# ChicyChen/LOCO-Edit

Hardware: AMD Instinct MI355X
Metric: edit-directions/sec (top-5 PMP-Jacobian SVD @256^2) + vT cos-sim vs ref (higher is better)
Workload: dtype bf16x3 (split-bf16 MFMA operands, fp32 accumulate + fp32 storage); 1 GPU; CelebA-HQ DDPM 256x256 top-5 local basis (l_eye-sized mask, L=2400), t=0.6T, 12 power iterations, one GPU; multi_gpu_form=single, probes_total=5, probes_per_gpu=5, kept=5, n_iter=12, mask_L=2400, weights=synthetic seed 0, streams=2

## Files before the change

### include/loco_hip.h

```cpp
#ifndef LOCO_HIP_H
#define LOCO_HIP_H

#include <stdint.h>

#ifdef __cplusplus
extern "C" {
#endif

typedef struct loco_ctx loco_ctx;

typedef struct loco_unet_cfg {
    int32_t struct_size;
    int32_t resolution;
    int32_t in_channels;
    int32_t out_ch;
    int32_t ch;
    int32_t num_levels;
    int32_t ch_mult[8];
    int32_t num_res_blocks;
    int32_t num_attn_res;
    int32_t attn_resolutions[8];
    int32_t gn_groups;
    float   gn_eps;
    int32_t max_batch;
// ... 33 lines not shown
int  loco_sched_step(loco_ctx* ctx, const float* x, const float* et, float at, float at_next,
                     float eta, const float* noise, int64_t count, float* x_next, float* x0_out,
                     void* stream);

int  loco_pmp_primal(loco_ctx* ctx, const float* x, float t, float at,
                     const uint8_t* mask, int32_t use_et, void* stream);
int  loco_pmp_set_second_mask(loco_ctx* ctx, const uint8_t* mask2, int32_t from_row, void* stream);
int  loco_pmp_jvp(loco_ctx* ctx, const float* V, int32_t k, float* U, void* stream);
int  loco_pmp_vjp(loco_ctx* ctx, const float* U, int32_t k, float* A, void* stream);

int  loco_orthonormalize(loco_ctx* ctx, float* A, int32_t k, int64_t n, float* s, void* stream);
int  loco_qr_rows(loco_ctx* ctx, float* A, int32_t k, int64_t n, void* stream);
int  loco_convergence(loco_ctx* ctx, const float* Vprev, const float* V, int64_t count,
                      float atol, float* out2, void* stream);
int  loco_convergence_rows(loco_ctx* ctx, const float* Vprev, const float* V, int32_t k, int64_t n,
                           float atol, float* out2, void* stream);

int  loco_null_project(loco_ctx* ctx, const float* Vm, int32_t k, const float* Vn, int32_t k0,
                       int64_t n, float* out, void* stream);
int  loco_edit_axpy(loco_ctx* ctx, const float* x, const float* v, const float* alphas,
                    int32_t B, int64_t n, float* out, void* stream);
int  loco_mask_gather(loco_ctx* ctx, const float* U, int32_t k, float* out, void* stream);
int64_t loco_mask_count(loco_ctx* ctx);

int  loco_clock_stamp(loco_ctx* ctx, uint64_t* out2, void* stream);

double loco_unet_flops(loco_ctx* ctx);
int64_t loco_workspace_bytes(loco_ctx* ctx);

int  loco_timer_start(loco_ctx* ctx, void* stream);
int  loco_timer_stop(loco_ctx* ctx, void* stream, float* ms);

int  loco_set_precision(loco_ctx* ctx, int32_t mode);
int  loco_set_streams(loco_ctx* ctx, int32_t n);
int  loco_set_side_stream(loco_ctx* ctx, void* stream);
int  loco_set_chip_share(loco_ctx* ctx, int32_t n);
int  loco_get_precision(loco_ctx* ctx);

int  loco_set_cond(loco_ctx* ctx, const float* emb_add, void* stream);
int  loco_set_time_cond(loco_ctx* ctx, const float* w_emb, void* stream);
int  loco_masked_axpby(loco_ctx* ctx, const float* V, const float* E, float cv, float ce, int32_t k, float* out,
                       void* stream);
int  loco_latent_sample(loco_ctx* ctx, const float* moments, const float* noise, float scale, int32_t B, float* z, void* stream);
int  loco_set_context(loco_ctx* ctx, const float* tokens, void* stream);

int  loco_lincomb(loco_ctx* ctx, const float* const* src, const float* coef, int32_t n, float* out, int64_t count,
// ... 147 lines not shown
```

### loco-edit_amd/csrc/engine.hip

```cpp
#include <hip/hip_runtime.h>

#include <algorithm>
#include <array>
#include <cmath>
#include <cstdio>
#include <cstdlib>
#include <cstring>
#include <map>
#include <memory>
#include <thread>
#include <atomic>
#include <string>
#include <vector>

#include "../../include/loco_hip.h"
#ifdef LOCO_DIAG
#include "../../include/loco_hip_diag.h"
#endif
#include "kernels.h"
#include "program.h"
#ifdef LOCO_DIAG
#include "conv_plan_text.h"
#endif

using namespace loco;


#define HIPCHK(ctx, call)                                                                    \
    do {                                                                                     \
        hipError_t e_ = (call);                                                              \
        if (e_ != hipSuccess) {                                                              \
            (ctx)->err = std::string(#call) + ": " + hipGetErrorString(e_);                  \
            return -1;                                                                       \
        }                                                                                    \
    } while (0)

namespace {

struct ConvP {
    float* wf = nullptr;
    float* wd = nullptr;
    float* wbf = nullptr;
// ... 77 lines not shown
    double *G = nullptr, *Q = nullptr, *W = nullptr, *gscratch = nullptr;
    float* alphas = nullptr;
    float* ctx_colbias = nullptr;
    bool has_ctx = false;
    float* cond_add = nullptr;
    float* ctx_norm = nullptr;
    bool has_cond = false;
    float* cond_in = nullptr;
    bool has_tcond = false;
    float2* sxcache = nullptr;
    int prec = 0;
    std::vector<float*> owned;
    size_t bytes = 0;

    bool primal_ok = false;
    float p_cv = 0.f, p_ce = 0.f;
    uint8_t* mask = nullptr;
    bool has_mask = false;
    uint8_t* mask2 = nullptr;
    bool has_mask2 = false;
    int mask2_from = 0;
    int* mask_idx = nullptr;
    int* mask_L_dev = nullptr;
    long mask_L = 0;
    hipStream_t mask_stream = nullptr;
    int primal_B = 0;
    hipEvent_t ev0 = nullptr, ev1 = nullptr;
    int n_streams = 1;
    hipStream_t st2 = nullptr;
    hipStream_t st2_user = nullptr;
    hipEvent_t ev_fork = nullptr, ev_join = nullptr;
    double* red2 = nullptr;
    struct FwdGraph { hipGraph_t graph = nullptr; hipGraphExec_t exec = nullptr; int calls = 0; };
    std::map<int, FwdGraph> fwd_graphs;
    bool graph_on = false;
    bool gemm_lowp = true;
    unsigned char* gemm_ws[2] = {nullptr, nullptr}; size_t gemm_ws_bytes[2] = {0, 0}; int lane = 0;
    loco_ctx* weights_of = nullptr;
    int forks = 0;
    bool zombie = false;
    bool fuse_lin = true;
    int lanes_active = 1;
    int lane_s0 = 0;
    int chip_share = 1;
    hipStream_t cap_st = nullptr;
    float* xin_buf = nullptr;
// ... 362 lines not shown
    if (c->prec >= 1 && c->gemm_lowp && gemm_prefers_bf16x3(g)) launch_gemm_bf16x3(g, st); else launch_gemm(g, st);
}

void conv_defaults(ConvArgs& a) {
    std::memset(&a, 0, sizeof(a));
    a.stride = 1; a.pad = 1; a.nsplit = 1; a.mode = CM_NONE; a.res_scale = 1.f;
}

struct NS { float *sc, *sh, *mr, *tst, *tc; };
NS nstats(const loco_ctx* c, float* base, const NormP& n) {
    NS s;
    s.sc = base + n.soff; s.sh = s.sc + n.C; s.mr = s.sh + n.C; s.tst = s.mr + 2 * c->cfg.gn_groups;
    s.tc = s.tst + 2 * c->cfg.gn_groups;
    return s;
}

struct StatReq {
    int kind = ST_NONE;
    NormP* n = nullptr;
    float* stats = nullptr;
    const float* prim = nullptr;
    const float* ss_scale = nullptr; const float* ss_shift = nullptr;
    float* keep = nullptr; size_t keep_floats = 0; int* keep_ntile = nullptr;
};

void stats_standalone(loco_ctx* c, const StatReq& rq, const float* x, long xbs, int B, int HW, int s0, hipStream_t st) {
    const NormP& n = *rq.n;
    const long SB = c->prog->stats_per_sample;
    const int G = c->cfg.gn_groups;
    if (rq.kind == ST_FWD) {
        NS s = nstats(c, rq.stats + (long)s0 * SB, n);
        launch_gn_stats(x, xbs, B, n.C, HW, G, eps_of(c, n), n.gamma, n.beta, s.mr, s.sc, s.sh, SB, c->red, st, rq.ss_scale,
                        rq.ss_shift);
    } else {
        NS sp = nstats(c, c->statsP, n);
        NS stt = nstats(c, rq.stats + (long)s0 * SB, n);
        launch_gn_tstats(x, xbs, rq.prim, 0, B, n.C, HW, G, sp.sc, sp.sh, sp.mr, 0, 0, rq.kind == ST_TAN ? 0 : 1, stt.tst,
                         stt.tc, SB, c->red, st, c->cfg.act);
    }
}

bool run_conv(loco_ctx* c, const ConvArgs& a0, int taps, hipStream_t st, const StatReq* rq = nullptr,
              const ConvArgs* second = nullptr) {
    const size_t span = (size_t)c->cfg.max_batch * c->prog->per_sample;
    auto padded = [&](const float* p) { return (p >= c->arenaP && p < c->arenaP + span) || (p >= c->arenaT && p < c->arenaT + span); };
    ConvArgs a = a0, sc;
    a.act = c->cfg.act;
    if (a.mode == CM_GN_SILU && c->cfg.act == ACT_GELU) a.mode = CM_GN_GELU;
    a.in_padded = padded(a.in);
    if (second) { sc = *second; sc.in_padded = padded(sc.in); }
    ConvEnv e;
    e.prec = c->prec; e.chip_share = c->chip_share; e.lanes = c->lanes_active; e.lane_s0 = c->lane_s0;
    e.partial = c->partial; e.partial_floats = c->partial_floats; e.stpart = c->stpart; e.stpart_floats = c->stpart_floats;
    e.fuse_stats = c->fuse_stats; e.fuse_lin = c->fuse_lin; e.deep1 = c->deep1; e.max_batch = c->cfg.max_batch;
    StatAsk q;
    if (rq) {
        q.kind = rq->kind; q.norm = rq->n != nullptr; q.prim = rq->prim; q.keep = rq->keep; q.keep_floats = rq->keep_floats;
        if (rq->n && rq->n->sx_off >= 0 && c->sxcache) q.sx = c->sxcache + rq->n->sx_off;
    }
    const ConvPlan p = plan_conv(e, a, taps, rq ? &q : nullptr, second ? &sc : nullptr);
    if (p.sc_first) run_conv(c, *second, 1, st);
#ifdef LOCO_DIAG
    if (c->plan_log) conv_plan_text(p, taps, c->prec, *c->plan_log);
#endif
    if (rq && rq->kind != ST_NONE && rq->n) rq->n->ready = true;
    if (rq && rq->keep_ntile) *rq->keep_ntile = p.keep_ntile;
    const int HWo = a.Hout * a.Wout, Gn = c->cfg.gn_groups;
    const long SBs = c->prog->stats_per_sample;
    auto timed = [&](const char* name, double flops, const ConvArgs& y, auto&& launch) {
        loco_ctx::ProfRec r;
        if (c->prof_on) {
            r.name = name; r.flops = flops;
            r.cin = y.Cin; r.cout = y.Cout; r.h = y.Hout; r.b = y.B; r.ns = y.nsplit; r.mode = y.mode; r.taps = taps;
            r.e0 = c->next_event(); r.e1 = c->next_event();
            (void)hipEventRecord(r.e0, st);
        }
        launch();
        if (c->prof_on) { (void)hipEventRecord(r.e1, st); c->prof.push_back(r); }
    };
    for (int li = 0; li < p.nl; ++li) {
        const ConvLaunch& l = p.l[li];
// ... 459 lines not shown
                a.out = p.T(op.out); a.out_bs = p.bs(); a.Cout = to.C; a.Hout = to.H; a.Wout = to.W; a.B = B;
                const StatReq rq = next_fwd(op.out);
                run_conv(c, a, 9, st, &rq);
                break;
            }
            case OP_OUT: {
                const Tens& ti = c->tens[op.in];
                if (!op.n1.ready) gn_forward_stats(p, op.n1, p.T(op.in), p.bs(), ti.H * ti.W);
                op.n1.ready = false;
                NS s = nstats(c, stats, op.n1);
                ConvArgs a; conv_defaults(a);
                a.in = p.T(op.in); a.in_bs = p.bs(); a.Cin = ti.C; a.Hin = ti.H; a.Win = ti.W;
                setw(a, op.conv, false); a.bias = op.conv.bias;
                a.mode = CM_GN_SILU; a.sc = s.sc; a.sh = s.sh; a.scsh_bs = SB;
                a.out = p.T(op.out); a.out_bs = p.bs(); a.Cout = to.C; a.Hout = to.H; a.Wout = to.W; a.B = B;
                run_conv(c, a, 9, st);
                break;
            }
        }
    }
    return 0;
}

void tangent_stats(loco_ctx* c, const NormP& n, const float* d, long dbs, const float* x, int HW, int B,
                   hipStream_t st) {
    NS sp = nstats(c, c->statsP, n);
    NS stt = nstats(c, c->statsT, n);
    launch_gn_tstats(d, dbs, x, 0, B, n.C, HW, c->cfg.gn_groups, sp.sc, sp.sh, sp.mr, 0, 0, 0, stt.tst,
                     stt.tc, c->prog->stats_per_sample, c->red, st);
}
void set_tan(loco_ctx* c, ConvArgs& a, const NormP& n, const float* prim) {
    NS sp = nstats(c, c->statsP, n);
    NS stt = nstats(c, c->statsT, n);
    a.mode = CM_TAN_SILU; a.prim = prim; a.prim_bs = 0;
    a.sc = sp.sc; a.sh = sp.sh; a.scsh_bs = 0; a.mr = sp.mr; a.mr_bs = 0; a.gamma_ = n.gamma;
    a.tst = stt.tst; a.tst_bs = c->prog->stats_per_sample; a.cpg = n.C / c->cfg.gn_groups;
    a.tc = stt.tc; a.tc_bs = c->prog->stats_per_sample;
    a.sx = (n.sx_off >= 0 && c->sxcache) ? c->sxcache + n.sx_off : nullptr;
}

constexpr size_t RED_BYTES = (size_t)4 << 20;

int tangent_pass(loco_ctx* c, const float* V, int B, hipStream_t st) {
    const loco_unet_cfg& cfg = c->cfg;
    const long PS = c->prog->per_sample;
    auto TP = [&](int id) { return c->arenaP + c->tens[id].off; };
// ... 145 lines not shown
                lin1x1(c, op.pj_out, false, XT_(X_H3), PS, C, TT(op.out), PS, C, H, W, B, TT(op.in), PS, false, st, &rq);
                break;
            }
            case OP_DOWN: case OP_UP: {
                const Tens& ti = c->tens[op.in];
                ConvArgs a; conv_defaults(a);
                a.in = TT(op.in); a.in_bs = PS; a.Cin = ti.C; a.Hin = ti.H; a.Win = ti.W;
                setw(a, op.conv, false);
                if (op.kind == OP_DOWN) { a.stride = 2; a.pad = op.sym_down ? 1 : 0; } else { a.upsample = 1; }
                a.out = TT(op.out); a.out_bs = PS; a.Cout = to.C; a.Hout = to.H; a.Wout = to.W; a.B = B;
                const StatReq rq = next_tan(op.out);
                run_conv(c, a, 9, st, &rq);
                break;
            }
            case OP_OUT: {
                const Tens& ti = c->tens[op.in];
                if (!op.n1.ready) tangent_stats(c, op.n1, TT(op.in), PS, TP(op.in), ti.H * ti.W, B, st);
                op.n1.ready = false;
                ConvArgs a; conv_defaults(a);
                a.in = TT(op.in); a.in_bs = PS; a.Cin = ti.C; a.Hin = ti.H; a.Win = ti.W;
                setw(a, op.conv, false);
                set_tan(c, a, op.n1, TP(op.in));
                a.out = TT(op.out); a.out_bs = PS; a.Cout = to.C; a.Hout = to.H; a.Wout = to.W; a.B = B;
                run_conv(c, a, 9, st);
                break;
            }
        }
    }
    return 0;
}

void cot_stats(loco_ctx* c, const NormP& n, const float* d, long dbs, const float* x, int HW, int B, int kind,
               hipStream_t st) {
    NS sp = nstats(c, c->statsP, n);
    NS stt = nstats(c, c->statsT, n);
    launch_gn_tstats(d, dbs, x, 0, B, n.C, HW, c->cfg.gn_groups, sp.sc, sp.sh, sp.mr, 0, 0, kind, stt.tst,
                     stt.tc, c->prog->stats_per_sample, c->red, st, c->cfg.act);
}

int cotangent_pass(loco_ctx* c, const float* ge, const float* gx0, float* Aout, int B, hipStream_t st) {
    const loco_unet_cfg& cfg = c->cfg;
    const long PS = c->prog->per_sample;
    const int G = cfg.gn_groups;
    auto TP = [&](int id) { return c->arenaP + c->tens[id].off; };
    auto TG = [&](int id) { return c->arenaT + c->tens[id].off; };
    auto GO = [&](const Op& o) -> const float* { return o.out == c->prog->eps_t ? ge : TG(o.out); };
    auto GOS = [&](const Op& o) -> long { return o.out == c->prog->eps_t ? (long)c->prog->n_out : PS; };
    clear_ready(c);
    for (int oi = (int)c->ops.size() - 1; oi >= 0; --oi) {
        Op& op = c->ops[oi];
        const Tens& to = c->tens[op.out];
        const int HW = to.H * to.W;
        switch (op.kind) {
            case OP_OUT: {
                const Tens& ti = c->tens[op.in];
                ConvArgs a; conv_defaults(a);
                a.in = GO(op); a.in_bs = GOS(op); a.Cin = to.C; a.Hin = to.H; a.Win = to.W;
                setw(a, op.conv, true);
                a.out = TG(op.a1); a.out_bs = PS; a.Cout = ti.C; a.Hout = ti.H; a.Wout = ti.W; a.B = B;
                {
                    const StatReq rq = req_lin(c, ST_COT, &op.n1, TP(op.in));
                    run_conv(c, a, 9, st, &rq);
                    op.n1.ready = false;
                }
                NS sp = nstats(c, c->statsP, op.n1);
                NS stt = nstats(c, c->statsT, op.n1);
                launch_gn_apply(2, TG(op.a1), PS, TP(op.in), 0, nullptr, 0, TG(op.in), PS, 0, B, ti.C, ti.H * ti.W, G,
                                sp.sc, sp.sh, sp.mr, 0, 0, stt.tst, c->prog->stats_per_sample, st, cfg.act);
                break;
            }
            case OP_UP: {
                const Tens& ti = c->tens[op.in];
                ConvArgs a; conv_defaults(a);
                a.in = TG(op.out); a.in_bs = PS; a.Cin = to.C; a.Hin = to.H; a.Win = to.W;
                setw(a, op.conv, true);
                a.out = TG(op.up); a.out_bs = PS; a.Cout = ti.C; a.Hout = to.H; a.Wout = to.W; a.B = B;
                run_conv(c, a, 9, st);
                launch_pool2x2_sum(TG(op.up), PS, TG(op.in), PS, 0, B, ti.C, ti.H, ti.W, st);
                break;
            }
            case OP_DOWN: {
                const Tens& ti = c->tens[op.in];
// ... 253 lines not shown
    }
    c->partial_floats = (size_t)64 << 20;
    if (dalloc(c, &c->partial, c->partial_floats)) return -1;
    if (dalloc(c, &c->xin_buf, MB * c->prog->n_in) || dalloc(c, &c->t_dev, 4)) return -1;
    if (dalloc(c, &c->eps_buf, MB * c->prog->n_out) || dalloc(c, &c->gx0, MB * c->prog->n_in) || dalloc(c, &c->ge, MB * c->prog->n_out))
        return -1;
    if (dalloc(c, &c->tmpA, (size_t)64 * c->prog->n_in)) return -1;
    if (dalloc(c, &c->G, 64 * 64) || dalloc(c, &c->Q, 64 * 64) || dalloc(c, &c->W, SOLVER_W_GATE + 1)) return -1;
    {
        size_t nblk = ((size_t)c->prog->n_in + 255) / 256;
        if (dalloc(c, &c->gscratch, nblk * 64 * 64 + 4096)) return -1;
    }
    if (dalloc(c, &c->alphas, 256) || dalloc(c, &c->cond_add, (size_t)cfg->ch * 4)) return -1;
    if (dalloc(c, &c->cond_in, (size_t)cfg->ch)) return -1;
    {
        float2* sx0 = nullptr;
        if (dalloc(c, &sx0, (size_t)c->prog->sx_total + 64)) return -1;
        c->sxcache = sx0 + 32;
    }
    {
        const char* e = getenv("LOCO_PRECISION");
        c->prec = (e && std::string(e) == "f32") ? 0 : (e && std::string(e) == "f16") ? 2 : 1;
    }
    if (dalloc(c, &c->mask2, (size_t)c->prog->n_out)) return -1;
    if (dalloc(c, &c->mask, (size_t)c->prog->n_out) || dalloc(c, &c->mask_idx, (size_t)c->prog->n_out) ||
        dalloc(c, &c->mask_L_dev, 4)) return -1;
    HIPCHK(c, hipEventCreate(&c->ev0));
    HIPCHK(c, hipEventCreate(&c->ev1));
    {
        const char* e = getenv("LOCO_STREAMS");
        c->n_streams = (e && atoi(e) == 2) ? 2 : 1;
        HIPCHK(c, hipStreamCreateWithFlags(&c->st2, hipStreamNonBlocking));
        HIPCHK(c, hipStreamCreateWithFlags(&c->cap_st, hipStreamNonBlocking));
        const char* gl = getenv("LOCO_GEMM_LOWP");
        if (gl) c->gemm_lowp = atoi(gl) != 0;
        const char* gr = getenv("LOCO_GRAPH");
        c->graph_on = gr && atoi(gr) == 1;
        HIPCHK(c, hipEventCreateWithFlags(&c->ev_fork, hipEventDisableTiming));
        HIPCHK(c, hipEventCreateWithFlags(&c->ev_join, hipEventDisableTiming));
    }
    return 0;
}

}

extern "C" {

const char* loco_version(void) { return "loco_hip 0.2 (gfx950; conv arithmetic: f32 MFMA | bf16x3 split-bf16 MFMA | f16 MFMA)"; }

// ... 141 lines not shown

int loco_sched_step(loco_ctx* c, const float* x, const float* et, float at, float at_next, float eta,
                    const float* noise, int64_t count, float* x_next, float* x0_out, void* stream) {
    if (!c) return -2;
    if (eta != 0.f && !noise) { c->err = "eta != 0 needs a noise tensor"; return -2; }
    float s1, s2, s3, ce, cn;
    sched_coeffs(at, at_next, eta, &s1, &s2, &s3, &ce, &cn);
    launch_ddim_step(x, et, eta == 0.f ? nullptr : noise, x_next, x0_out, (long)count, s2, s1, s3, ce, cn,
                     (hipStream_t)stream);
    HIPCHK(c, hipGetLastError());
    return 0;
}

int loco_ddim_step(loco_ctx* c, const float* x, float t, float at, float at_next, float eta, const float* noise,
                   int32_t B, float* x_next, void* stream) {
    if (!c) return -2;
    if (eta != 0.f && !noise) { c->err = "eta != 0 needs a noise tensor"; return -2; }
    if (c->prog->n_out != c->prog->n_in) { c->err = "loco_ddim_step: this network is not a denoiser (output and input sizes differ)"; return -2; }
    int rc = loco_unet_forward(c, x, t, B, c->eps_buf, stream);
    if (rc) return rc;
    return loco_sched_step(c, x, c->eps_buf, at, at_next, eta, noise, (int64_t)B * c->prog->n_in, x_next, nullptr, stream);
}

int loco_pmp_primal(loco_ctx* c, const float* x, float t, float at, const uint8_t* mask, int32_t use_et,
                    void* stream) {
    if (!c) return -2;
    if (finalize_params(c)) return -3;
    if (c->prog->n_out != c->prog->n_in && !use_et) {
        c->err = "loco_pmp_primal: a network whose output size differs from its input has no x0 combination; use_et = 1 "
                 "(raw network Jacobian)";
        return -2;
    }
    hipStream_t st = (hipStream_t)stream;
    if (forward_pass(c, x, t, 1, c->arenaP, c->statsP, st)) return -1;
    c->primal_B = 1;
    if (c->prec >= 1) {
        for (auto& op : c->ops) {
            if (op.kind != OP_RES && op.kind != OP_OUT) continue;
            const Tens& ti = c->tens[op.in];
            const int HW = ti.H * ti.W, G = c->cfg.gn_groups;
            NS s1 = nstats(c, c->statsP, op.n1);
            launch_gn_cache(c->arenaP + ti.off, op.n1.C, HW, op.n1.C / G, s1.sc, s1.sh, s1.mr,
                            c->sxcache + op.n1.sx_off, st, c->cfg.act);
            if (op.kind == OP_RES) {
                const Tens& th = c->tens[op.h1];
                NS s2 = nstats(c, c->statsP, op.n2);
                launch_gn_cache(c->arenaP + th.off, op.n2.C, th.H * th.W, op.n2.C / G, s2.sc, s2.sh, s2.mr,
                                c->sxcache + op.n2.sx_off, st, c->cfg.act);
            }
        }
    }
    if (use_et) { c->p_cv = 0.f; c->p_ce = 1.f; }
    else { c->p_cv = 1.0f / std::sqrt(at); c->p_ce = -std::sqrt(1.0f - at) / std::sqrt(at); }
    c->has_mask = (mask != nullptr);
    c->has_mask2 = false;
    c->mask_L = c->prog->n_out;
    if (mask) {
        HIPCHK(c, hipMemcpyAsync(c->mask, mask, (size_t)c->prog->n_out, hipMemcpyDeviceToDevice, st));
        launch_mask_compact(c->mask, c->prog->n_out, c->mask_idx, c->mask_L_dev, st);
        c->mask_L = -1;
        c->mask_stream = st;
    }
    HIPCHK(c, hipGetLastError());
    c->primal_ok = true;
    return 0;
}

int loco_pmp_set_second_mask(loco_ctx* c, const uint8_t* mask2, int32_t from_row, void* stream) {
    if (!c) return -2;
    if (!c->primal_ok) { c->err = "loco_pmp_primal has not been called"; return -2; }
    if (!mask2) { c->has_mask2 = false; return 0; }
    if (!c->has_mask) { c->err = "a second mask needs a first one (loco_pmp_primal with mask)"; return -2; }
    if (from_row < 0) { c->err = "from_row must be >= 0"; return -2; }
    HIPCHK(c, hipMemcpyAsync(c->mask2, mask2, (size_t)c->prog->n_out, hipMemcpyDeviceToDevice, (hipStream_t)stream));
    c->has_mask2 = true;
    c->mask2_from = from_row;
    return 0;
}

int loco_pmp_jvp(loco_ctx* c, const float* V, int32_t k, float* U, void* stream) {
    if (!c) return -2;
    if (!c->primal_ok) { c->err = "loco_pmp_primal has not been called"; return -2; }
    hipStream_t st = (hipStream_t)stream;
    const int MB = c->cfg.max_batch;
    for (int b0 = 0; b0 < k; b0 += MB) {
        int B = (k - b0 < MB) ? k - b0 : MB;
        int rc = run_lanes(c, B, st, [&](int s0, int nb, hipStream_t ls) -> int {
            const float* Vc = V + (long)(b0 + s0) * c->prog->n_in;
            if (tangent_pass(c, Vc, nb, ls)) return -1;
            launch_copy(c->arenaT + c->tens[c->prog->eps_t].off, c->prog->per_sample, c->eps_buf, c->prog->n_out, 0, nb, c->prog->n_out, ls);
            launch_masked_axpby(c->prog->n_out == c->prog->n_in ? Vc : nullptr, c->eps_buf, c->has_mask ? c->mask : nullptr, c->p_cv,
                                c->p_ce, U + (long)(b0 + s0) * c->prog->n_out, nb, c->prog->n_out, ls,
                                c->has_mask2 ? c->mask2 : nullptr, (long)c->mask2_from - (b0 + s0));
            return 0;
        });
        if (rc) return rc;
    }
    HIPCHK(c, hipGetLastError());
    return 0;
// ... 636 lines not shown
```

### loco-edit_amd/csrc/kernels.h

```cpp
#pragma once
#include <hip/hip_runtime.h>
#include <stdint.h>

namespace loco {

struct DeviceOnce { bool seen[64] = {}; };
inline bool first_on_device(DeviceOnce& f) {
    int d = 0;
    (void)hipGetDevice(&d);
    d &= 63;
    if (f.seen[d]) return false;
    f.seen[d] = true;
    return true;
}


enum ConvMode : int {
    CM_NONE = 0,
    CM_GN_SILU = 1,
    CM_GN = 2,
    CM_TAN_SILU = 3,
    CM_COT_SILU = 4,
    CM_GN_GELU = 5,
};
// ... 241 lines not shown
                       hipStream_t st, const double* gate = nullptr);
constexpr int SOLVER_W_GATE = 64;
constexpr double SOLVER_W_FLOOR = 0x1p-47;
constexpr double SOLVER_REORTHO_RATIO = 1e-7;
void launch_jacobi_eig(double* G, int k, double* w, double* Q, hipStream_t st);
void launch_rotate_rows(const float* Ain, float* Aout, int k, long n, const double* Q, const double* w,
                        int mode, hipStream_t st);
void launch_sign_fix(float* A, int k, long n, float* s_out, const double* w, float* scratch, hipStream_t st);
void launch_cholesky(double* G, int k, hipStream_t st, double drop_below = 0.0, double* w = nullptr,
                     const double* gate = nullptr);
void launch_trsm_rows(const float* Ain, float* Aout, int k, long n, const double* L, hipStream_t st,
                      const double* gate = nullptr);
void launch_convergence(const float* a, const float* b, long count, float atol, float rtol, float* out2,
                        double* scratch, hipStream_t st);
void launch_convergence_rows(const float* a, const float* b, int k, long n, float atol, float rtol, float* out2,
                             double* scratch, hipStream_t st);
void launch_project_rows(const float* Vm, int k, const float* Vn, int k0, long n, const double* C,
                         float* out, hipStream_t st);
void launch_normalize_rows(float* A, int k, long n, double* scratch, hipStream_t st);
void launch_edit_axpy(const float* x, const float* v, const float* alphas_dev, int B, long n, float* out,
                      hipStream_t st);
void launch_mask_gather(const float* U, const int* idx, long L, long n, int k, float* out, hipStream_t st);
void launch_mask_compact(const uint8_t* mask, long n, int* idx, int* count, hipStream_t st);

}
```

### loco-edit_amd/csrc/misc.hip

```cpp
#include "kernels.h"

namespace loco {

typedef float f32x4_t __attribute__((ext_vector_type(4)));

__device__ __forceinline__ double wave_sum(double v) {
#pragma unroll
    for (int o = 32; o > 0; o >>= 1) v += __shfl_down(v, o, 64);
    return v;
}
__device__ __forceinline__ float wave_sumf(float v) {
#pragma unroll
    for (int o = 32; o > 0; o >>= 1) v += __shfl_down(v, o, 64);
    return v;
}
__device__ __forceinline__ float wave_maxf(float v) {
#pragma unroll
    for (int o = 32; o > 0; o >>= 1) v = fmaxf(v, __shfl_down(v, o, 64));
    return v;
}
__device__ __forceinline__ double block_sum(double v, double* sm) {
    v = wave_sum(v);
    __syncthreads();
    if ((threadIdx.x & 63) == 0) sm[threadIdx.x >> 6] = v;
// ... 826 lines not shown
}

__global__ void copy_kernel(const float* in, long in_bs, float* out, long out_bs, int accumulate, long per) {
    const int b = blockIdx.y;
    for (long i = ((long)blockIdx.x * blockDim.x + threadIdx.x) * 4; i < per; i += (long)gridDim.x * blockDim.x * 4) {
        float4 v = *reinterpret_cast<const float4*>(in + (long)b * in_bs + i);
        float4* o = reinterpret_cast<float4*>(out + (long)b * out_bs + i);
        if (accumulate) {
            float4 w = *o;
            v.x += w.x; v.y += w.y; v.z += w.z; v.w += w.w;
        }
        *o = v;
    }
}
void launch_copy(const float* in, long in_bs, float* out, long out_bs, int accumulate, int B, long per_sample,
                 hipStream_t st) {
    int blocks = (int)((per_sample / 4 + 255) / 256);
    if (blocks > 2048) blocks = 2048;
    if (blocks < 1) blocks = 1;
    hipLaunchKernelGGL(copy_kernel, dim3(blocks, B), dim3(256), 0, st, in, in_bs, out, out_bs, accumulate,
                       per_sample);
}

__global__ void ddim_step_kernel(const float* x, const float* eps, const float* noise, float* out, float* x0_out,
                                 long count, float sq1mat, float sqat, float sqatn, float ce, float cn) {
    for (long i = (long)blockIdx.x * blockDim.x + threadIdx.x; i < count; i += (long)gridDim.x * blockDim.x) {
        float e = eps[i];
        float p = (x[i] - e * sq1mat) / sqat;
        float v = sqatn * p + ce * e;
        if (noise) v += cn * noise[i];
        if (x0_out) x0_out[i] = p;
        out[i] = v;
    }
}
void launch_ddim_step(const float* x, const float* eps, const float* noise, float* out, float* x0_out, long count,
                      float c_x0_x, float c_x0_e, float c_next_x0, float c_next_e, float c_noise, hipStream_t st) {
    int blocks = (int)((count + 255) / 256);
    if (blocks > 2048) blocks = 2048;
    hipLaunchKernelGGL(ddim_step_kernel, dim3(blocks), dim3(256), 0, st, x, eps, noise, out, x0_out, count, c_x0_e, c_x0_x,
                       c_next_x0, c_next_e, c_noise);
}

__global__ void masked_axpby_kernel(const float* V, const float* dE, const uint8_t* mask, float cv, float ce,
                                    float* U, long n, long total, const uint8_t* mask2, long split) {
    for (long i = (long)blockIdx.x * blockDim.x + threadIdx.x; i < total; i += (long)gridDim.x * blockDim.x) {
        long row = i / n, j = i - row * n;
// ... 99 lines not shown
```

### loco-edit_amd/csrc/solver.hip

```cpp
#include "kernels.h"

namespace loco {

constexpr int GCH = 256;

__device__ __forceinline__ double wsum(double v) {
#pragma unroll
    for (int o = 32; o > 0; o >>= 1) v += __shfl_down(v, o, 64);
    return v;
}

__global__ __launch_bounds__(256) void cross_gram_partial(const float* A, int k1, const float* B, int k2, long n,
                                                          double* part, const double* gate) {
    extern __shared__ float sm[];
    if (gate && *gate == 0.0) return;
    float* As = sm;
    float* Bs = sm + (long)k1 * (GCH + 1);
    const long c0 = (long)blockIdx.x * GCH;
    for (int e = threadIdx.x; e < k1 * GCH; e += 256) {
        int i = e / GCH, c = e % GCH;
        As[i * (GCH + 1) + c] = (c0 + c < n) ? A[(long)i * n + c0 + c] : 0.f;
    }
    if (B != A) {
        for (int e = threadIdx.x; e < k2 * GCH; e += 256) {
// ... 463 lines not shown
    const long per = (n + 1023) / 1024;
    const long lo = (long)t * per, hi = lo + per < n ? lo + per : n;
    int cnt = 0;
    for (long i = lo; i < hi; ++i) cnt += mask[i] != 0;
    int inc = cnt;
#pragma unroll
    for (int o = 1; o < 64; o <<= 1) {
        int v = __shfl_up(inc, o, 64);
        if (lane >= o) inc += v;
    }
    if (lane == 63) wtot[wv] = inc;
    __syncthreads();
    int base = 0;
    for (int w = 0; w < wv; ++w) base += wtot[w];
    int pos = base + inc - cnt;
    for (long i = lo; i < hi; ++i)
        if (mask[i]) idx[pos++] = (int)i;
    if (t == 1023) *count = base + inc;
}
void launch_mask_compact(const uint8_t* mask, long n, int* idx, int* count, hipStream_t st) {
    hipLaunchKernelGGL(mask_compact_kernel, dim3(1), dim3(1024), 0, st, mask, n, idx, count);
}

}
```

### loco-edit_amd/hip.py

```python
from __future__ import annotations

import ctypes as C
import os
from typing import Dict, Optional

import numpy as np
import torch

from .config import UNetConfig

_LIB_PATH = os.environ.get("LOCO_HIP_LIB") or os.path.join(os.path.dirname(os.path.abspath(__file__)), "libloco_hip.so")
_lib = None

DIAG_SYMBOLS = ["loco_bench_conv", "loco_debug_conv", "loco_debug_tensor"]

SYMBOLS = [
    "loco_version", "loco_device_count", "loco_create", "loco_fork", "loco_destroy", "loco_last_error",
    "loco_load_param", "loco_params_missing", "loco_unet_forward", "loco_ddim_step", "loco_sched_step",
    "loco_pmp_primal", "loco_pmp_set_second_mask", "loco_pmp_jvp", "loco_pmp_vjp", "loco_orthonormalize", "loco_qr_rows",
    "loco_convergence", "loco_convergence_rows", "loco_null_project", "loco_edit_axpy", "loco_mask_gather", "loco_mask_count",
    "loco_unet_flops", "loco_workspace_bytes", "loco_clock_stamp", "loco_set_side_stream", "loco_timer_start", "loco_timer_stop",
    "loco_profile_enable", "loco_profile_report", "loco_set_precision", "loco_get_precision", "loco_set_streams", "loco_set_chip_share",
    "loco_set_cond", "loco_set_context", "loco_lincomb", "loco_masked_axpby", "loco_latent_sample",
    "loco_text_create", "loco_text_load_param", "loco_text_params_missing", "loco_text_encode", "loco_text_last_error",
    "loco_text_destroy", "loco_t5_create", "loco_text_encode_masked",
    "loco_diffedit_mask", "loco_cfg_masked_step", "loco_set_time_cond", "loco_lcm_step",
    "loco_sam_create", "loco_sam_load_param", "loco_sam_params_missing", "loco_sam_encode", "loco_sam_profile",
    "loco_sam_profile_read", "loco_sam_last_error", "loco_sam_destroy",
    "loco_samdec_create", "loco_samdec_load_param", "loco_samdec_params_missing", "loco_samdec_set_image", "loco_samdec_predict",
    "loco_samdec_score", "loco_samdec_binarize", "loco_samdec_last_error", "loco_samdec_destroy",
    "loco_clipvis_create", "loco_clipvis_load_param", "loco_clipvis_params_missing", "loco_clipvis_preprocess",
    "loco_clipvis_encode", "loco_clipvis_last_error", "loco_clipvis_destroy",
    "loco_quality_create", "loco_quality_load_param", "loco_quality_params_missing", "loco_quality_lpips", "loco_quality_ssim",
    "loco_quality_masked_mse", "loco_quality_last_error", "loco_quality_destroy",
]

DIFFEDIT_RULES = {"reference": 0, "intended": 1}


class LocoCfg(C.Structure):
    _fields_ = [
        ("struct_size", C.c_int32), ("resolution", C.c_int32), ("in_channels", C.c_int32), ("out_ch", C.c_int32), ("ch", C.c_int32),
        ("num_levels", C.c_int32), ("ch_mult", C.c_int32 * 8), ("num_res_blocks", C.c_int32),
# ... 76 lines not shown
        lib.loco_fork.argtypes = [vp, C.c_int32, C.POINTER(vp)]
    lib.loco_destroy.argtypes = [vp]
    lib.loco_destroy.restype = None
    lib.loco_last_error.argtypes = [vp]
    lib.loco_last_error.restype = C.c_char_p
    lib.loco_load_param.argtypes = [vp, C.c_char_p, vp, C.POINTER(i64), i32, i32]
    lib.loco_params_missing.argtypes = [vp]
    lib.loco_unet_forward.argtypes = [vp, vp, f32, i32, vp, vp]
    lib.loco_ddim_step.argtypes = [vp, vp, f32, f32, f32, f32, vp, i32, vp, vp]
    lib.loco_sched_step.argtypes = [vp, vp, vp, f32, f32, f32, vp, i64, vp, vp, vp]
    lib.loco_pmp_primal.argtypes = [vp, vp, f32, f32, vp, i32, vp]
    lib.loco_pmp_set_second_mask.argtypes = [vp, vp, i32, vp]
    lib.loco_pmp_jvp.argtypes = [vp, vp, i32, vp, vp]
    lib.loco_pmp_vjp.argtypes = [vp, vp, i32, vp, vp]
    lib.loco_orthonormalize.argtypes = [vp, vp, i32, i64, vp, vp]
    lib.loco_qr_rows.argtypes = [vp, vp, i32, i64, vp]
    lib.loco_convergence.argtypes = [vp, vp, vp, i64, f32, vp, vp]
    lib.loco_convergence_rows.argtypes = [vp, vp, vp, i32, i64, f32, vp, vp]
    lib.loco_null_project.argtypes = [vp, vp, i32, vp, i32, i64, vp, vp]
    lib.loco_edit_axpy.argtypes = [vp, vp, vp, C.POINTER(f32), i32, i64, vp, vp]
    lib.loco_mask_gather.argtypes = [vp, vp, i32, vp, vp]
    lib.loco_mask_count.argtypes = [vp]
    lib.loco_mask_count.restype = i64
    lib.loco_clock_stamp.argtypes = [vp, vp, vp]
    lib.loco_set_side_stream.argtypes = [vp, vp]
    lib.loco_unet_flops.argtypes = [vp]
    lib.loco_unet_flops.restype = C.c_double
    lib.loco_workspace_bytes.argtypes = [vp]
    lib.loco_workspace_bytes.restype = i64
    lib.loco_timer_start.argtypes = [vp, vp]
    lib.loco_timer_stop.argtypes = [vp, vp, C.POINTER(f32)]
    lib.loco_set_precision.argtypes = [vp, i32]
    lib.loco_get_precision.argtypes = [vp]
    lib.loco_set_streams.argtypes = [vp, i32]
    lib.loco_set_chip_share.argtypes = [vp, i32]
    lib.loco_set_cond.argtypes = [vp, vp, vp]
    lib.loco_set_context.argtypes = [vp, vp, vp]
    lib.loco_masked_axpby.argtypes = [vp, vp, vp, f32, f32, i32, vp, vp]
    lib.loco_latent_sample.argtypes = [vp, vp, vp, f32, i32, vp, vp]
    lib.loco_lincomb.argtypes = [vp, C.POINTER(vp), C.POINTER(f32), i32, vp, i64, vp]
    lib.loco_diffedit_mask.argtypes = [vp, vp, vp, f32, i32, i32, i64, i32, vp, vp, vp]
    lib.loco_cfg_masked_step.argtypes = [vp, vp, vp, vp, vp, f32, f32, f32, vp, i32, i64, vp, vp]
    lib.loco_set_time_cond.argtypes = [vp, vp, vp]
    lib.loco_lcm_step.argtypes = [vp, vp, vp, f32, f32, f32, f32, vp, i64, vp, vp, vp]
    lib.loco_profile_enable.argtypes = [vp, i32]
    lib.loco_profile_report.argtypes = [vp, C.c_char_p, i64]
# ... 293 lines not shown
    def edit_axpy(self, x, v, alphas) -> torch.Tensor:
        _chk_dev(x)
        _chk_dev(v)
        B = len(alphas)
        n = x.numel()
        out = torch.empty((B,) + tuple(x.shape[1:]), device=x.device, dtype=torch.float32)
        arr = (C.c_float * B)(*[float(a) for a in alphas])
        self._check(self.lib.loco_edit_axpy(self._ctx, _ptr(x), _ptr(v), arr, B, n, _ptr(out), _stream()),
                    "loco_edit_axpy")
        torch.cuda.current_stream().synchronize()
        return out

    def mask_gather(self, U) -> torch.Tensor:
        _chk_dev(U)
        k = U.shape[0]
        L = int(self.lib.loco_mask_count(self._ctx))
        out = torch.empty(k, L, device=U.device, dtype=torch.float32)
        self._check(self.lib.loco_mask_gather(self._ctx, _ptr(U), k, _ptr(out), _stream()), "loco_mask_gather")
        return out

    def mask_count(self) -> int:
        return int(self.lib.loco_mask_count(self._ctx))

    def set_cond(self, emb_add: Optional[torch.Tensor]):
        if emb_add is not None:
            _chk_dev(emb_add)
            if emb_add.numel() != 4 * self.cfg.ch:
                raise ValueError("conditioning embedding must have 4*ch elements")
        self._check(self.lib.loco_set_cond(self._ctx, _ptr(emb_add), _stream()), "loco_set_cond")

    def set_time_cond(self, w_emb: Optional[torch.Tensor]):
        if w_emb is not None:
            _chk_dev(w_emb)
            if self.cfg.time_cond_proj_dim > 0 and w_emb.numel() != self.cfg.time_cond_proj_dim:
                raise ValueError(f"guidance-scale embedding must have time_cond_proj_dim = {self.cfg.time_cond_proj_dim} "
                                 f"elements, got {tuple(w_emb.shape)}")
        self._check(self.lib.loco_set_time_cond(self._ctx, _ptr(w_emb), _stream()), "loco_set_time_cond")
        if w_emb is not None:
            torch.cuda.current_stream().synchronize()

    def set_context(self, tokens: torch.Tensor):
        _chk_dev(tokens)
        if tuple(tokens.shape) != (self.cfg.context_len, self.cfg.context_dim):
            raise ValueError(f"context must be [{self.cfg.context_len}, {self.cfg.context_dim}], got {tuple(tokens.shape)}")
        self._check(self.lib.loco_set_context(self._ctx, _ptr(tokens), _stream()), "loco_set_context")
        torch.cuda.current_stream().synchronize()
# ... 544 lines not shown
```

Before: 19.79 edit-directions/s.

## Restrict final output conv JVP/VJP to a window around the mask bounding box

Computes the mask's bounding box once after the primal pass and picks an aligned square window (H/4 or H/2) covering it plus a one-pixel halo. The last output conv in the tangent (JVP) and cotangent (VJP) passes then runs only on that window: inputs, primal activations and split-precision caches are copied into it, and the results are scattered back. For the VJP, GroupNorm tangent stats are rescaled by the window-to-full-area ratio and a windowed GN-backward apply kernel fills the full tensor. This removes full-resolution work on the costly final conv at the price of extra copies, a host sync during primal setup, and some numerical risk in the stats rescaling.

```diff
diff --git a/include/loco_hip.h b/include/loco_hip.h
--- a/include/loco_hip.h
+++ b/include/loco_hip.h
@@ -79,6 +79,7 @@
                     int32_t B, int64_t n, float* out, void* stream);
 int  loco_mask_gather(loco_ctx* ctx, const float* U, int32_t k, float* out, void* stream);
 int64_t loco_mask_count(loco_ctx* ctx);
+int  loco_mask_window(loco_ctx* ctx, int32_t out[3]);
 
 int  loco_clock_stamp(loco_ctx* ctx, uint64_t* out2, void* stream);
 
diff --git a/loco-edit_amd/csrc/engine.hip b/loco-edit_amd/csrc/engine.hip
--- a/loco-edit_amd/csrc/engine.hip
+++ b/loco-edit_amd/csrc/engine.hip
@@ -18,6 +18,7 @@
 #include "../../include/loco_hip_diag.h"
 #endif
 #include "kernels.h"
+#include "mask_window.h"
 #include "program.h"
 #ifdef LOCO_DIAG
 #include "conv_plan_text.h"
@@ -141,6 +142,10 @@
     int mask2_from = 0;
     int* mask_idx = nullptr;
     int* mask_L_dev = nullptr;
+    MaskWindow win;
+    float* win_buf = nullptr; size_t win_floats = 0;
+    float *win_prim = nullptr, *win_big = nullptr, *win_small = nullptr;
+    float2* win_sx = nullptr;
     long mask_L = 0;
     hipStream_t mask_stream = nullptr;
     int primal_B = 0;
@@ -549,6 +554,7 @@
     const float* prim = nullptr;
     const float* ss_scale = nullptr; const float* ss_shift = nullptr;
     float* keep = nullptr; size_t keep_floats = 0; int* keep_ntile = nullptr;
+    const float2* sx = nullptr;
 };
 
 void stats_standalone(loco_ctx* c, const StatReq& rq, const float* x, long xbs, int B, int HW, int s0, hipStream_t st) {
@@ -570,7 +576,10 @@
 bool run_conv(loco_ctx* c, const ConvArgs& a0, int taps, hipStream_t st, const StatReq* rq = nullptr,
               const ConvArgs* second = nullptr) {
     const size_t span = (size_t)c->cfg.max_batch * c->prog->per_sample;
-    auto padded = [&](const float* p) { return (p >= c->arenaP && p < c->arenaP + span) || (p >= c->arenaT && p < c->arenaT + span); };
+    auto padded = [&](const float* p) {
+        return (p >= c->arenaP && p < c->arenaP + span) || (p >= c->arenaT && p < c->arenaT + span) ||
+               (c->win_buf && p >= c->win_buf && p < c->win_buf + c->win_floats);
+    };
     ConvArgs a = a0, sc;
     a.act = c->cfg.act;
     if (a.mode == CM_GN_SILU && c->cfg.act == ACT_GELU) a.mode = CM_GN_GELU;
@@ -583,7 +592,8 @@
     StatAsk q;
     if (rq) {
         q.kind = rq->kind; q.norm = rq->n != nullptr; q.prim = rq->prim; q.keep = rq->keep; q.keep_floats = rq->keep_floats;
-        if (rq->n && rq->n->sx_off >= 0 && c->sxcache) q.sx = c->sxcache + rq->n->sx_off;
+        if (rq->sx) q.sx = rq->sx;
+        else if (rq->n && rq->n->sx_off >= 0 && c->sxcache) q.sx = c->sxcache + rq->n->sx_off;
     }
     const ConvPlan p = plan_conv(e, a, taps, rq ? &q : nullptr, second ? &sc : nullptr);
     if (p.sc_first) run_conv(c, *second, 1, st);
@@ -1089,6 +1099,10 @@
     return 0;
 }
 
+inline bool window_on(const loco_ctx* c, const Op& op) {
+    return c->win.S > 0 && !c->has_mask2 && op.kind == OP_OUT && op.out == c->prog->eps_t && &op == &c->ops.back();
+}
+
 void tangent_stats(loco_ctx* c, const NormP& n, const float* d, long dbs, const float* x, int HW, int B,
                    hipStream_t st) {
     NS sp = nstats(c, c->statsP, n);
@@ -1280,6 +1294,19 @@
                 setw(a, op.conv, false);
                 set_tan(c, a, op.n1, TP(op.in));
                 a.out = TT(op.out); a.out_bs = PS; a.Cout = to.C; a.Hout = to.H; a.Wout = to.W; a.B = B;
+                if (window_on(c, op)) {
+                    const MaskWindow& w = c->win;
+                    const long in_ws = (long)ti.C * w.S * w.S, out_ws = (long)to.C * w.S * w.S;
+                    float* tin = c->win_big + c->lane_s0 * in_ws;
+                    float* tout = c->win_small + c->lane_s0 * out_ws;
+                    launch_window_copy(1, TT(op.in), PS, tin, in_ws, B, ti.C, ti.H, ti.W, w.y0, w.x0, w.S, w.S, st);
+                    a.in = tin; a.in_bs = in_ws; a.Hin = a.Win = w.S;
+                    a.prim = c->win_prim; if (a.sx) a.sx = c->win_sx;
+                    a.out = tout; a.out_bs = out_ws; a.Hout = a.Wout = w.S;
+                    run_conv(c, a, 9, st);
+                    launch_window_copy(0, tout, out_ws, TT(op.out), PS, B, to.C, to.H, to.W, w.y0, w.x0, w.S, w.S, st);
+                    break;
+                }
                 run_conv(c, a, 9, st);
                 break;
             }
@@ -1316,6 +1343,26 @@
                 a.in = GO(op); a.in_bs = GOS(op); a.Cin = to.C; a.Hin = to.H; a.Win = to.W;
                 setw(a, op.conv, true);
                 a.out = TG(op.a1); a.out_bs = PS; a.Cout = ti.C; a.Hout = ti.H; a.Wout = ti.W; a.B = B;
+                if (window_on(c, op)) {
+                    const MaskWindow& w = c->win;
+                    const long in_ws = (long)to.C * w.S * w.S, out_ws = (long)ti.C * w.S * w.S;
+                    float* seed = c->win_small + c->lane_s0 * in_ws;
+                    float* a1w = c->win_big + c->lane_s0 * out_ws;
+                    launch_window_copy(1, GO(op), GOS(op), seed, in_ws, B, to.C, to.H, to.W, w.y0, w.x0, w.S, w.S, st);
+                    a.in = seed; a.in_bs = in_ws; a.Hin = a.Win = w.S;
+                    a.out = a1w; a.out_bs = out_ws; a.Hout = a.Wout = w.S;
+                    StatReq rq = req_lin(c, ST_COT, &op.n1, c->win_prim);
+                    if (c->prec >= 1) rq.sx = c->win_sx;
+                    run_conv(c, a, 9, st, &rq);
+                    op.n1.ready = false;
+                    NS sp = nstats(c, c->statsP, op.n1);
+                    NS stt = nstats(c, c->statsT, op.n1);
+                    launch_scale_rows(stt.tst, c->prog->stats_per_sample, B, 2 * G + 2 * ti.C,
+                                      (float)(w.S * w.S) / (float)(ti.H * ti.W), st);
+                    launch_gn_apply_window(a1w, out_ws, TP(op.in), TG(op.in), PS, B, ti.C, ti.H, ti.W, w.y0, w.x0, w.S, G, sp.sc,
+                                           sp.sh, sp.mr, stt.tst, c->prog->stats_per_sample, st, cfg.act);
+                    break;
+                }
                 {
                     const StatReq rq = req_lin(c, ST_COT, &op.n1, TP(op.in));
                     run_conv(c, a, 9, st, &rq);
@@ -1615,9 +1662,21 @@
         const char* e = getenv("LOCO_PRECISION");
         c->prec = (e && std::string(e) == "f32") ? 0 : (e && std::string(e) == "f16") ? 2 : 1;
     }
+    if (!c->ops.empty() && c->ops.back().kind == OP_OUT) {
+        const Tens& to = c->tens[c->ops.back().out];
+        const Tens& ti = c->tens[c->ops.back().in];
+        MaskWindowAsk q;
+        q.C = to.C; q.H = to.H; q.W = to.W; q.has_mask = true; q.out_conv3 = true; q.y0 = q.x0 = q.y1 = q.x1 = 0;
+        if (choose_mask_window(q).S > 0 && ti.H == to.H && ti.W == to.W) {
+            const size_t S2 = (size_t)(to.H / 2) * (to.H / 2), MBw = (size_t)c->cfg.max_batch, PAD = 64;
+            c->win_floats = PAD + ti.C * S2 + PAD + 2 * ti.C * S2 + PAD + MBw * ti.C * S2 + PAD + MBw * to.C * S2 + PAD;
+            if (dalloc(c, &c->win_buf, c->win_floats)) return -1;
+            HIPCHK(c, hipMemset(c->win_buf, 0, c->win_floats * sizeof(float)));
+        }
+    }
     if (dalloc(c, &c->mask2, (size_t)c->prog->n_out)) return -1;
     if (dalloc(c, &c->mask, (size_t)c->prog->n_out) || dalloc(c, &c->mask_idx, (size_t)c->prog->n_out) ||
-        dalloc(c, &c->mask_L_dev, 4)) return -1;
+        dalloc(c, &c->mask_L_dev, 8)) return -1;
     HIPCHK(c, hipEventCreate(&c->ev0));
     HIPCHK(c, hipEventCreate(&c->ev1));
     {
@@ -1805,6 +1864,49 @@
     return loco_sched_step(c, x, c->eps_buf, at, at_next, eta, noise, (int64_t)B * c->prog->n_in, x_next, nullptr, stream);
 }
 
+static int window_setup(loco_ctx* c, hipStream_t st) {
+    const char* e = getenv("LOCO_MASK_WINDOW");
+    if (e && atoi(e) == 0) return 0;
+    const Program& P = *c->prog;
+    if (c->ops.empty()) return 0;
+    const Op& op = c->ops.back();
+    const Tens& to = c->tens[op.out];
+    MaskWindowAsk q;
+    q.C = to.C; q.H = to.H; q.W = to.W;
+    q.has_mask = c->has_mask; q.second_mask = c->has_mask2;
+    q.out_conv3 = op.kind == OP_OUT && op.out == P.eps_t && op.conv.taps == 9 && (long)to.C * to.H * to.W == P.n_out &&
+                  c->tens[op.in].H == to.H && c->tens[op.in].W == to.W;
+    {
+        MaskWindowAsk t = q;
+        t.y0 = t.x0 = t.y1 = t.x1 = 0;
+        if (choose_mask_window(t).S == 0) return 0;
+    }
+    hipStreamCaptureStatus cs = hipStreamCaptureStatusNone;
+    if (hipStreamIsCapturing(st, &cs) != hipSuccess || cs != hipStreamCaptureStatusNone) return 0;
+    launch_mask_bbox(c->mask, to.C, to.H, to.W, c->mask_L_dev + 4, st);
+    int host[8] = {0, 0, 0, 0, 0, 0, -1, -1};
+    HIPCHK(c, hipMemcpyAsync(host, c->mask_L_dev, sizeof(host), hipMemcpyDeviceToHost, st));
+    HIPCHK(c, hipStreamSynchronize(st));
+    c->mask_L = host[0];
+    q.y0 = host[4]; q.x0 = host[5]; q.y1 = host[6]; q.x1 = host[7];
+    const MaskWindow w = choose_mask_window(q);
+    if (w.S == 0) return 0;
+    const Tens& ti = c->tens[op.in];
+    const size_t S2 = (size_t)w.S * w.S, MB = (size_t)c->cfg.max_batch, PAD = 64;
+    const size_t need = PAD + ti.C * S2 + PAD + 2 * ti.C * S2 + PAD + MB * ti.C * S2 + PAD + MB * to.C * S2 + PAD;
+    if (need > c->win_floats) return 0;
+    c->win_prim = c->win_buf + PAD;
+    c->win_sx = reinterpret_cast<float2*>(c->win_prim + ti.C * S2 + PAD);
+    c->win_big = reinterpret_cast<float*>(c->win_sx) + 2 * ti.C * S2 + PAD;
+    c->win_small = c->win_big + MB * ti.C * S2 + PAD;
+    launch_window_copy(1, c->arenaP + ti.off, 0, c->win_prim, 0, 1, ti.C, ti.H, ti.W, w.y0, w.x0, w.S, w.S, st);
+    if (c->prec >= 1 && op.n1.sx_off >= 0)
+        launch_window_copy(1, reinterpret_cast<const float*>(c->sxcache + op.n1.sx_off), 0, reinterpret_cast<float*>(c->win_sx), 0, 1,
+                           ti.C, ti.H, 2 * ti.W, w.y0, 2 * w.x0, w.S, 2 * w.S, st);
+    c->win = w;
+    return 0;
+}
+
 int loco_pmp_primal(loco_ctx* c, const float* x, float t, float at, const uint8_t* mask, int32_t use_et,
                     void* stream) {
     if (!c) return -2;
@@ -1844,8 +1946,17 @@
         c->mask_L = -1;
         c->mask_stream = st;
     }
+    c->win = MaskWindow();
+    if (mask && window_setup(c, st)) return -1;
     HIPCHK(c, hipGetLastError());
     c->primal_ok = true;
+    return 0;
+}
+
+int loco_mask_window(loco_ctx* c, int32_t out[3]) {
+    if (!c || !out) return -2;
+    const bool on = c->primal_ok && c->win.S > 0 && !c->has_mask2;
+    out[0] = on ? c->win.y0 : 0; out[1] = on ? c->win.x0 : 0; out[2] = on ? c->win.S : 0;
     return 0;
 }
 
@@ -1858,6 +1969,7 @@
     HIPCHK(c, hipMemcpyAsync(c->mask2, mask2, (size_t)c->prog->n_out, hipMemcpyDeviceToDevice, (hipStream_t)stream));
     c->has_mask2 = true;
     c->mask2_from = from_row;
+    c->win.S = 0;
     return 0;
 }
 
diff --git a/loco-edit_amd/csrc/kernels.h b/loco-edit_amd/csrc/kernels.h
--- a/loco-edit_amd/csrc/kernels.h
+++ b/loco-edit_amd/csrc/kernels.h
@@ -287,5 +287,13 @@
                       hipStream_t st);
 void launch_mask_gather(const float* U, const int* idx, long L, long n, int k, float* out, hipStream_t st);
 void launch_mask_compact(const uint8_t* mask, long n, int* idx, int* count, hipStream_t st);
-
-}
+void launch_mask_bbox(const uint8_t* mask, int C, int H, int W, int* box, hipStream_t st);
+
+void launch_window_copy(int to_window, const float* src, long src_bs, float* dst, long dst_bs, int B, int C, int H, int W, int y0,
+                        int x0, int SH, int SW, hipStream_t st);
+void launch_gn_apply_window(const float* dw, long dw_bs, const float* x, float* out, long out_bs, int B, int C, int H, int W, int y0,
+                            int x0, int S, int G, const float* sc, const float* sh, const float* mr, const float* tst, long tst_bs,
+                            hipStream_t st, int act);
+void launch_scale_rows(float* p, long bs, int B, int count, float f, hipStream_t st);
+
+}
diff --git a/loco-edit_amd/csrc/mask_window.h b/loco-edit_amd/csrc/mask_window.h
--- /dev/null
+++ b/loco-edit_amd/csrc/mask_window.h
@@ -0,0 +1,20 @@
+#pragma once
+
+namespace loco {
+
+struct MaskWindowAsk {
+    int C = 0, H = 0, W = 0;
+    bool has_mask = false;
+    bool second_mask = false;
+    bool out_conv3 = false;
+    int y0 = 0, x0 = 0, y1 = -1, x1 = -1;
+};
+
+struct MaskWindow { int y0 = 0, x0 = 0, S = 0; };
+
+constexpr int kMaskWindowMinSide = 8;
+constexpr int kMaskWindowAlignX = 4;
+
+MaskWindow choose_mask_window(const MaskWindowAsk& q);
+
+}
diff --git a/loco-edit_amd/csrc/mask_window.hip b/loco-edit_amd/csrc/mask_window.hip
--- /dev/null
+++ b/loco-edit_amd/csrc/mask_window.hip
@@ -0,0 +1,29 @@
+#include "mask_window.h"
+
+namespace loco {
+
+MaskWindow choose_mask_window(const MaskWindowAsk& q) {
+    MaskWindow none;
+    if (!q.has_mask || q.second_mask || !q.out_conv3) return none;
+    if (q.C < 1 || q.H < 1 || q.H != q.W) return none;
+    if (q.y1 < q.y0 || q.x1 < q.x0) return none;
+    if (q.y0 < 0 || q.x0 < 0 || q.y1 >= q.H || q.x1 >= q.W) return none;
+    const int gy0 = q.y0 > 0 ? q.y0 - 1 : 0, gx0 = q.x0 > 0 ? q.x0 - 1 : 0;
+    const int gy1 = q.y1 + 1 < q.H ? q.y1 + 1 : q.H - 1, gx1 = q.x1 + 1 < q.W ? q.x1 + 1 : q.W - 1;
+    for (int div = 4; div >= 2; div -= 2) {
+        if (q.H % (div * kMaskWindowAlignX) != 0) continue;
+        const int S = q.H / div;
+        if (S < kMaskWindowMinSide) continue;
+        int y0 = gy0, x0 = gx0 - gx0 % kMaskWindowAlignX;
+        if (y0 > q.H - S) y0 = q.H - S;
+        if (x0 > q.W - S) x0 = q.W - S;
+        if (gy1 < y0 + S && gx1 < x0 + S) {
+            MaskWindow w;
+            w.y0 = y0; w.x0 = x0; w.S = S;
+            return w;
+        }
+    }
+    return none;
+}
+
+}
diff --git a/loco-edit_amd/csrc/misc.hip b/loco-edit_amd/csrc/misc.hip
--- a/loco-edit_amd/csrc/misc.hip
+++ b/loco-edit_amd/csrc/misc.hip
@@ -872,6 +872,88 @@
                        per_sample);
 }
 
+template <int TO_WINDOW>
+__global__ __launch_bounds__(256) void window_copy_kernel(const float* src, long src_bs, float* dst, long dst_bs, int C, int HW,
+                                                          int W, int y0, int x0, int SH, int SW) {
+    const int b = blockIdx.y;
+    const int q = SW >> 2;
+    const long units = (long)C * SH * q;
+    for (long u = (long)blockIdx.x * 256 + threadIdx.x; u < units; u += (long)gridDim.x * 256) {
+        const int c = (int)(u / ((long)SH * q));
+        const int r = (int)(u - (long)c * SH * q);
+        const int yy = r / q, xq = r - yy * q;
+        const long full = (long)c * HW + (long)(y0 + yy) * W + x0 + 4 * xq;
+        const long win = 4 * u;
+        if (TO_WINDOW) *reinterpret_cast<float4*>(dst + (long)b * dst_bs + win) = *reinterpret_cast<const float4*>(src + (long)b * src_bs + full);
+        else *reinterpret_cast<float4*>(dst + (long)b * dst_bs + full) = *reinterpret_cast<const float4*>(src + (long)b * src_bs + win);
+    }
+}
+void launch_window_copy(int to_window, const float* src, long src_bs, float* dst, long dst_bs, int B, int C, int H, int W, int y0,
+                        int x0, int SH, int SW, hipStream_t st) {
+    const long units = (long)C * SH * (SW / 4);
+    int blocks = (int)((units + 255) / 256);
+    if (blocks > 2048) blocks = 2048;
+    if (blocks < 1) blocks = 1;
+    if (to_window)
+        hipLaunchKernelGGL(window_copy_kernel<1>, dim3(blocks, B), dim3(256), 0, st, src, src_bs, dst, dst_bs, C, H * W, W, y0, x0, SH, SW);
+    else
+        hipLaunchKernelGGL(window_copy_kernel<0>, dim3(blocks, B), dim3(256), 0, st, src, src_bs, dst, dst_bs, C, H * W, W, y0, x0, SH, SW);
+}
+
+__global__ __launch_bounds__(256) void gn_apply_window_kernel(const float* dw, long dw_bs, const float* x, float* out, long out_bs,
+                                                              int C, int HW, int W, int y0, int x0, int S, int cpg, const float* sc,
+                                                              const float* sh, const float* mr, const float* tst, long tbs, int act) {
+    const int b = blockIdx.y;
+    const long per = (long)C * HW;
+    for (long i = ((long)blockIdx.x * 256 + threadIdx.x) * 4; i < per; i += (long)gridDim.x * 1024) {
+        const int c = (int)(i / HW);
+        const int p = (int)(i - (long)c * HW);
+        const int y = p / W, xc = p - y * W;
+        const int g = c / cpg;
+        const float scc = sc[c], shc = sh[c];
+        const float mean = mr[2 * g], rstd = mr[2 * g + 1];
+        const float m1 = tst[(long)b * tbs + g * 2], m2 = tst[(long)b * tbs + g * 2 + 1];
+        const float4 xv = *reinterpret_cast<const float4*>(x + i);
+        const float xx[4] = {xv.x, xv.y, xv.z, xv.w};
+        float r[4];
+        const int wy = y - y0, wx = xc - x0;
+        if (wy >= 0 && wy < S && wx >= 0 && wx < S) {
+            const float4 dv = *reinterpret_cast<const float4*>(dw + (long)b * dw_bs + ((long)c * S + wy) * S + wx);
+            const float dd[4] = {dv.x, dv.y, dv.z, dv.w};
+            const float gm = scc / rstd;
+#pragma unroll
+            for (int j = 0; j < 4; ++j) {
+                const float xh = (xx[j] - mean) * rstd;
+                r[j] = rstd * (gm * act_der(fmaf(scc, xx[j], shc), act) * dd[j] - m1 - xh * m2);
+            }
+        } else {
+#pragma unroll
+            for (int j = 0; j < 4; ++j) {
+                const float xh = (xx[j] - mean) * rstd;
+                r[j] = rstd * (0.f - m1 - xh * m2);
+            }
+        }
+        *reinterpret_cast<float4*>(out + (long)b * out_bs + i) = make_float4(r[0], r[1], r[2], r[3]);
+    }
+}
+void launch_gn_apply_window(const float* dw, long dw_bs, const float* x, float* out, long out_bs, int B, int C, int H, int W, int y0,
+                            int x0, int S, int G, const float* sc, const float* sh, const float* mr, const float* tst, long tst_bs,
+                            hipStream_t st, int act) {
+    const long per = (long)C * H * W;
+    int blocks = (int)((per / 4 + 255) / 256);
+    if (blocks > 1024) blocks = 1024;
+    hipLaunchKernelGGL(gn_apply_window_kernel, dim3(blocks, B), dim3(256), 0, st, dw, dw_bs, x, out, out_bs, C, H * W, W, y0, x0, S,
+                       C / G, sc, sh, mr, tst, tst_bs, act);
+}
+
+__global__ void scale_rows_kernel(float* p, long bs, int count, float f) {
+    const int i = blockIdx.x * blockDim.x + threadIdx.x;
+    if (i < count) p[(long)blockIdx.y * bs + i] *= f;
+}
+void launch_scale_rows(float* p, long bs, int B, int count, float f, hipStream_t st) {
+    hipLaunchKernelGGL(scale_rows_kernel, dim3((count + 255) / 256, B), dim3(256), 0, st, p, bs, count, f);
+}
+
 __global__ void ddim_step_kernel(const float* x, const float* eps, const float* noise, float* out, float* x0_out,
                                  long count, float sq1mat, float sqat, float sqatn, float ce, float cn) {
     for (long i = (long)blockIdx.x * blockDim.x + threadIdx.x; i < count; i += (long)gridDim.x * blockDim.x) {
diff --git a/loco-edit_amd/csrc/solver.hip b/loco-edit_amd/csrc/solver.hip
--- a/loco-edit_amd/csrc/solver.hip
+++ b/loco-edit_amd/csrc/solver.hip
@@ -509,4 +509,25 @@
     hipLaunchKernelGGL(mask_compact_kernel, dim3(1), dim3(1024), 0, st, mask, n, idx, count);
 }
 
-}
+__global__ __launch_bounds__(1024) void mask_bbox_kernel(const uint8_t* mask, int HW, int W, long n, int* box) {
+    __shared__ int ext[4];
+    const int t = threadIdx.x;
+    if (t == 0) { ext[0] = HW / W; ext[1] = W; ext[2] = -1; ext[3] = -1; }
+    __syncthreads();
+    const long per = (n + 1023) / 1024;
+    const long lo = (long)t * per, hi = lo + per < n ? lo + per : n;
+    int y0 = 0x7fffffff, x0 = 0x7fffffff, y1 = -1, x1 = -1;
+    for (long i = lo; i < hi; ++i) {
+        if (!mask[i]) continue;
+        const int p = (int)(i % HW), y = p / W, x = p - y * W;
+        y0 = y < y0 ? y : y0; x0 = x < x0 ? x : x0; y1 = y > y1 ? y : y1; x1 = x > x1 ? x : x1;
+    }
+    if (y1 >= 0) { atomicMin(&ext[0], y0); atomicMin(&ext[1], x0); atomicMax(&ext[2], y1); atomicMax(&ext[3], x1); }
+    __syncthreads();
+    if (t < 4) box[t] = ext[t];
+}
+void launch_mask_bbox(const uint8_t* mask, int C, int H, int W, int* box, hipStream_t st) {
+    hipLaunchKernelGGL(mask_bbox_kernel, dim3(1), dim3(1024), 0, st, mask, H * W, W, (long)C * H * W, box);
+}
+
+}
diff --git a/loco-edit_amd/hip.py b/loco-edit_amd/hip.py
--- a/loco-edit_amd/hip.py
+++ b/loco-edit_amd/hip.py
@@ -18,7 +18,7 @@
     "loco_version", "loco_device_count", "loco_create", "loco_fork", "loco_destroy", "loco_last_error",
     "loco_load_param", "loco_params_missing", "loco_unet_forward", "loco_ddim_step", "loco_sched_step",
     "loco_pmp_primal", "loco_pmp_set_second_mask", "loco_pmp_jvp", "loco_pmp_vjp", "loco_orthonormalize", "loco_qr_rows",
-    "loco_convergence", "loco_convergence_rows", "loco_null_project", "loco_edit_axpy", "loco_mask_gather", "loco_mask_count",
+    "loco_convergence", "loco_convergence_rows", "loco_null_project", "loco_edit_axpy", "loco_mask_gather", "loco_mask_count", "loco_mask_window",
     "loco_unet_flops", "loco_workspace_bytes", "loco_clock_stamp", "loco_set_side_stream", "loco_timer_start", "loco_timer_stop",
     "loco_profile_enable", "loco_profile_report", "loco_set_precision", "loco_get_precision", "loco_set_streams", "loco_set_chip_share",
     "loco_set_cond", "loco_set_context", "loco_lincomb", "loco_masked_axpby", "loco_latent_sample",
@@ -141,6 +141,7 @@
     lib.loco_mask_gather.argtypes = [vp, vp, i32, vp, vp]
     lib.loco_mask_count.argtypes = [vp]
     lib.loco_mask_count.restype = i64
+    lib.loco_mask_window.argtypes = [vp, vp]
     lib.loco_clock_stamp.argtypes = [vp, vp, vp]
     lib.loco_set_side_stream.argtypes = [vp, vp]
     lib.loco_unet_flops.argtypes = [vp]
@@ -480,6 +481,11 @@
     def mask_count(self) -> int:
         return int(self.lib.loco_mask_count(self._ctx))
 
+    def mask_window(self):
+        out = (C.c_int32 * 3)()
+        self._check(self.lib.loco_mask_window(self._ctx, out), "loco_mask_window")
+        return int(out[0]), int(out[1]), int(out[2])
+
     def set_cond(self, emb_add: Optional[torch.Tensor]):
         if emb_add is not None:
             _chk_dev(emb_add)
```

After: 19.95 edit-directions/s, median of 6. No clear change (+0.8%).
